# ma-compbio/MATCHA

Measured on AMD Instinct MI355X. Metric: training hyperedges/sec at k∈{2..5}, embed_dim=64; 1/2/4/8 MI355X, higher is better.
Workload: dtype f32; 1 GPU; hg38_1mb bins (N=3067), k in {2,3,4,5} mixed-k zero-padded to L=5, embed_dim=64, front end=table, neg_num=3, dropout on, AdamW lr=1e-3, 400000 known hyperedges; parallelism=dp1, hipgraph=False, table_gradient_exchange=none, embedding_backward=float atomics, exchange_overlapped=False

## Files before the change

### include/matcha_hip.h

```cpp
#ifndef MATCHA_HIP_H
#define MATCHA_HIP_H

#include <stddef.h>
#include <stdint.h>

#ifdef __cplusplus
extern "C" {
#endif

#define MATCHA_ABI_VERSION 7

#define MATCHA_OK 0
#define MATCHA_EINVAL (-22)
#define MATCHA_EHIP (-5)
#define MATCHA_ENOMEM (-12)

#define MATCHA_MAX_L 8
#define MATCHA_MAX_LONG_L 32
#define MATCHA_N_HEAD 8

typedef void* matcha_stream_t;

int matcha_abi_version(void);
const char* matcha_last_error(void);
int matcha_device_count(void);

#define MATCHA_PROF_GEMM_NT 1
#define MATCHA_PROF_GEMM_NN 2
#define MATCHA_PROF_GEMM_TN 3
#define MATCHA_PROF_ATTN_FWD 4
#define MATCHA_PROF_ATTN_BWD 5
#define MATCHA_PROF_EMBED_FWD 6
#define MATCHA_PROF_EMBED_SCATTER 7
#define MATCHA_PROF_LN3_FWD 8
#define MATCHA_PROF_LN3_BWD 9
#define MATCHA_PROF_HEAD_FWD 10
#define MATCHA_PROF_HEAD_BWD 11
#define MATCHA_PROF_ADAMW 12
#define MATCHA_PROF_NEG_SAMPLE 13
#define MATCHA_PROF_ADJ_ENCODE 14
#define MATCHA_PROF_GATHER_ROWS 15
#define MATCHA_PROF_FUSED_FWD 16
#define MATCHA_PROF_FUSED_BWD 17
#define MATCHA_PROF_FRONT_FWD 18
#define MATCHA_PROF_FRONT_BWD 19
#define MATCHA_PROF_ADJ_RECON 20
#define MATCHA_PROF_ADJ_BWD 21
int matcha_profile_select(int32_t kernel_class);
int matcha_profile_read(double* total_ms, int64_t* launches, double* work);

int matcha_launch_log(int32_t on);
int matcha_launch_log_read(char* out, size_t cap);

int matcha_set_option(const char* name, int32_t value);
int32_t matcha_get_option(const char* name);

#define MATCHA_STATUS_BAD_ID 1
#define MATCHA_STATUS_BAD_CHROM 2

typedef struct matcha_shape {
  int32_t d;
  int32_t n_attr;
  int32_t n_nodes;
  int32_t n_chrom;
  int32_t mode;
  int32_t max_bins;
} matcha_shape;

typedef struct matcha_tensors {
  float* table;
  float* adj_w0;
  float* adj_w1;
  float* recon_w;
  float* recon_b;
  float* attr_w;
  float* attr_b;
  float* next_w;
  float* next_b;
  float* ln_q_g; float* ln_q_b;
  float* ln_k_g; float* ln_k_b;
  float* ln_v_g; float* ln_v_b;
  float* w_q;
  float* w_k;
  float* w_v;
  float* fc1_w;
// ... 328 lines not shown
```

### matcha_amd/_lib.py

```python
from __future__ import annotations

import ctypes as C
import os

_HERE = os.path.dirname(os.path.abspath(__file__))
LIB_PATH = os.environ.get("MATCHA_HIP_LIB") or os.path.join(_HERE, "lib", "libmatcha_hip.so")

MAX_L = 8
MAX_LONG_L = 32
N_HEAD = 8

GEMM_NT, GEMM_NN, GEMM_TN = 0, 1, 2
EPI_BIAS, EPI_TANH, EPI_DROPOUT, EPI_ROWMASK, EPI_RESIDUAL, EPI_DTANH, EPI_ACCUM = 1, 2, 4, 8, 16, 32, 64

PROF = dict(gemm_nt=1, gemm_nn=2, gemm_tn=3, attn_fwd=4, attn_bwd=5, embed_fwd=6, embed_scatter=7, ln3_fwd=8, ln3_bwd=9,
            head_fwd=10, head_bwd=11, adamw=12, neg_sample=13, adj_encode=14, gather_rows=15, fused_fwd=16, fused_bwd=17, front_fwd=18, front_bwd=19,
            adj_recon=20, adj_bwd=21)

_fp = C.c_void_p


class Shape(C.Structure):
    _fields_ = [("d", C.c_int32), ("n_attr", C.c_int32), ("n_nodes", C.c_int32), ("n_chrom", C.c_int32),
                ("mode", C.c_int32), ("max_bins", C.c_int32)]
# ... 12 lines not shown
class Frozen(C.Structure):
    _fields_ = [("attr_table", _fp), ("bounds", _fp), ("feats", _fp), ("feat_off", _fp), ("inter", _fp),
                ("bounds_host", _fp), ("feat_row_pad", C.c_int32), ("attr_mode", C.c_int32), ("attr_ld", C.c_int32),
                ("attr_scale", C.c_float), ("attr_bounds", _fp)]


class StepOpts(C.Structure):
    _fields_ = [("training", C.c_int32), ("random_chrom", C.c_int32), ("p_drop_adj", C.c_float),
                ("p_drop_fc1", C.c_float), ("p_drop_pff", C.c_float), ("alpha", C.c_float), ("beta", C.c_float),
                ("seed", _fp), ("forward_only", C.c_int32), ("loss_in_forward", C.c_int32), ("status", _fp),
                ("sparse_table_grad", C.c_int32), ("deterministic", C.c_int32), ("encoder_done_event", _fp),
                ("random_chrom_dev", _fp)]


class RaggedView(C.Structure):
    _fields_ = [("row_off", _fp), ("tok_slot", _fp), ("tok_id", _fp), ("tok_key", _fp), ("tok_pos", _fp), ("count", _fp),
                ("tile_meta", _fp), ("tiles_cap", C.c_int64), ("half_meta", _fp), ("halves_cap", C.c_int64), ("tok_tile", _fp)]


class GemmEpilogue(C.Structure):
    _fields_ = [("flags", C.c_int32), ("bias", _fp), ("residual", _fp), ("aux", _fp), ("row_ids", _fp), ("seed", _fp),
                ("stream_id", C.c_int32), ("p_drop", C.c_float), ("aux_scale", C.c_float)]


_I64, _I32, _SZ, _D, _F = C.c_int64, C.c_int32, C.c_size_t, C.c_double, C.c_float
SIGNATURES = {
    "matcha_abi_version": (C.c_int, []),
    "matcha_last_error": (C.c_char_p, []),
    "matcha_device_count": (C.c_int, []),
    "matcha_profile_select": (C.c_int, [_I32]),
    "matcha_profile_read": (C.c_int, [C.POINTER(C.c_double), C.POINTER(C.c_int64), C.POINTER(C.c_double)]),
    "matcha_launch_log": (C.c_int, [_I32]),
    "matcha_launch_log_read": (C.c_int, [C.c_char_p, _SZ]),
    "matcha_workspace_bytes": (_SZ, [C.POINTER(Shape), _I64, _I32]),
    "matcha_workspace_bytes_forward": (_SZ, [C.POINTER(Shape), _I64, _I32]),
    "matcha_forward": (C.c_int, [C.POINTER(Shape), C.POINTER(Tensors), C.POINTER(Frozen), C.POINTER(StepOpts), _fp, _I64,
                                 _I32, _fp, _fp, _fp, _fp, _fp, _SZ, _fp]),
    "matcha_workspace_bytes_long": (_SZ, [C.POINTER(Shape), _I64, _I32]),
    "matcha_forward_long": (C.c_int, [C.POINTER(Shape), C.POINTER(Tensors), C.POINTER(Frozen), C.POINTER(StepOpts), _fp, _I64,
                                      _I32, _fp, _fp, _fp, _SZ, _fp]),
    "matcha_get_embedding_long": (C.c_int, [C.POINTER(Shape), C.POINTER(Tensors), C.POINTER(Frozen), C.POINTER(StepOpts), _fp, _I64, _I32,
                                            _fp, _fp, _fp, _fp, _fp, _SZ, _fp]),
    "matcha_workspace_bytes_long_train": (_SZ, [C.POINTER(Shape), _I64, _I32]),
    "matcha_forward_long_train": (C.c_int, [C.POINTER(Shape), C.POINTER(Tensors), C.POINTER(Frozen), C.POINTER(StepOpts), _fp, _I64,
                                            _I32, _fp, _fp, _fp, _SZ, _fp]),
    "matcha_backward_long": (C.c_int, [C.POINTER(Shape), C.POINTER(Tensors), C.POINTER(Frozen), C.POINTER(StepOpts), _fp, _I64,
                                       _I32, _fp, _fp, C.POINTER(Tensors), _fp, _fp, _SZ, _fp]),
    "matcha_attn_long_bwd_workspace_bytes": (_SZ, [_I64, _I32]),
    "matcha_attn_long_bwd": (C.c_int, [_fp, _fp, _fp, _fp, _fp, _I64, _I32, _I32, _I32, _fp, _fp, _fp, _fp, _SZ, _fp]),
    "matcha_backward": (C.c_int, [C.POINTER(Shape), C.POINTER(Tensors), C.POINTER(Frozen), C.POINTER(StepOpts), _fp, _I64,
                                  _I32, _fp, _fp, _fp, _fp, C.POINTER(Tensors), _fp, _fp, _SZ, _fp]),
    "matcha_forward_objective": (C.c_int, [_I32, C.POINTER(Shape), C.POINTER(Tensors), C.POINTER(Frozen), C.POINTER(StepOpts), _fp, _I64,
                                           _I32, _fp, _fp, _fp, _fp, _fp, _SZ, _fp]),
    "matcha_backward_objective": (C.c_int, [_I32, C.POINTER(Shape), C.POINTER(Tensors), C.POINTER(Frozen), C.POINTER(StepOpts), _fp, _I64,
                                            _I32, _fp, _fp, _fp, _fp, C.POINTER(Tensors), _fp, _fp, _SZ, _fp]),
    "matcha_node_embeddings": (C.c_int, [C.POINTER(Shape), C.POINTER(Tensors), C.POINTER(Frozen), _fp, _I64, _fp, _fp, _SZ, _fp, _fp]),
    "matcha_get_embedding": (C.c_int, [C.POINTER(Shape), C.POINTER(Tensors), C.POINTER(Frozen), C.POINTER(StepOpts), _fp, _I64, _I32,
                                       _fp, _fp, _fp, _fp, _fp, _SZ, _fp]),
    "matcha_table_grad_rows": (C.c_int, [C.POINTER(Shape), _I64, _I32, _fp, _SZ, C.POINTER(C.c_void_p), C.POINTER(C.c_void_p),
                                         C.POINTER(C.c_void_p), C.POINTER(C.c_int64)]),
    "matcha_scatter_rows_workspace_bytes": (_SZ, [_I64, _I32, _I32]),
    "matcha_scatter_rows": (C.c_int, [_fp, _fp, _I64, _I32, _I32, _fp, _fp, _SZ, _fp]),
    "matcha_ragged_plan_bytes": (_SZ, [_I64, _I32]),
    "matcha_ragged_plan": (C.c_int, [_fp, _I64, _I32, _I32, _fp, _fp, _SZ, C.POINTER(RaggedView), _fp]),
    "matcha_random_chrom_dev_supported": (C.c_int, [C.POINTER(Shape), C.POINTER(Frozen)]),
    "matcha_set_option": (C.c_int, [C.c_char_p, _I32]),
# ... 137 lines not shown
    return old


class option:

    def __init__(self, name: str, value: int = 1):
        self.name, self.value = name, value

    def __enter__(self):
        self.old = set_option(self.name, self.value)
        return self

    def __exit__(self, *a):
        set_option(self.name, self.old)


class launch_log:

    def __enter__(self):
        self.counts = {}
        check(load().matcha_launch_log(1), "matcha_launch_log")
        return self

    def __exit__(self, *a):
        lib = load()
        lib.matcha_launch_log(0)
        buf = C.create_string_buffer(1 << 14)
        check(lib.matcha_launch_log_read(buf, len(buf)), "matcha_launch_log_read")
        for line in buf.value.decode().splitlines():
            name, n = line.rsplit(" ", 1)
            self.counts[name] = int(n)


def raise_on_status(status_host, what: str):
    if status_host[0] & STATUS_BAD_ID:
        raise IndexError(f"{what}: node id outside [0, n_nodes] (the reference's nn.Embedding raises 'index out of range in self')")
    if status_host[0] & STATUS_BAD_CHROM:
        raise KeyError(f"{what}: a node without a chromosome (node2chrom < 0) reached the negative sampler")
```

### matcha_amd/csrc/fused_fwd32.hip

```cpp
#include "kernels.hpp"
#include "prep_heads.hpp"
#include "ragged_roles.hpp"

#ifndef F32_ABL
#define F32_ABL 0
#endif

namespace matcha {

typedef float f32x16 __attribute__((ext_vector_type(16)));

namespace {

constexpr int kLdH = 68;
constexpr int kHT = 32 * kLdH;
constexpr float kEps32 = 1e-5f;
constexpr int kTailVec32 = 2 * 4096;
constexpr int kTailSlab32 = 2 * 4096 + 10 * 64;

struct FL { f32x16 lo, hi; };

__device__ __forceinline__ float xhalf_sum(float v) {
  float a = v, b = v;
  asm volatile("s_nop 1\n\tv_permlane32_swap_b32 %0, %1" : "+v"(a), "+v"(b));
// ... 158 lines not shown
  } while (0)

__device__ __forceinline__ FL fl_zero() {
  FL v;
#pragma unroll
  for (int e = 0; e < 16; ++e) { v.lo[e] = 0.f; v.hi[e] = 0.f; }
  return v;
}

}

__global__ __launch_bounds__(256) void prep_heads_kernel(PrepArgs a) {
  __shared__ __attribute__((aligned(16))) float sm[kPrepLdsFloats];
  prep_heads_role(a, blockIdx.x, blockIdx.y, blockIdx.z, sm);
}

struct Fwd32Args {
  const float* X;
  const int32_t* xrow;
  const int32_t* row_off; const int32_t* tok_slot; const int32_t* count; const int32_t* half_meta; const int32_t* tok_pos;
  int L;
  const u32x4* wfrag;
  HeadParams hp;
  const float* y; const float* w;
  float* Y; float* H1; float* H2;
  float* logits; float* row_loss;
  const uint64_t* seed;
  float p_fc1, p_pff;
  float* ddyn0; float* dXs; float* tslab; float alpha_over_B;
  int objective;
  float* qkv;
  float* tail_dh2;
  const float* rn;
  int rn_rows;
  float* dxs_node;
};

template <int ML>
__global__ __launch_bounds__(64) __attribute__((amdgpu_waves_per_eu(2, 2))) void fused_fwd32_kernel(Fwd32Args g) {
  extern __shared__ __attribute__((aligned(16))) float lds[];
#ifdef FF_TIMING
  long long tph[16] = {0};
  long long tlast = wall_clock64();
#define FF_T(i) do { const long long now__ = wall_clock64(); tph[i] += now__ - tlast; tlast = now__; } while (0)
#else
#define FF_T(i) do { } while (0)
#endif
  float* TK = lds;
  float* TV = lds + kHT;
  float* outs = lds + 2 * kHT;
  float* douts = outs + 32;
  const int lane = threadIdx.x, r = lane & 31, h = lane >> 5;

  const int4 meta = reinterpret_cast<const int4*>(g.half_meta)[blockIdx.x];
  const int t0 = meta.x, n = meta.y, b0 = meta.z, n_h = meta.w;
  if (n_h <= 0) return;
  const int tok_pad = g.count[1];
  const float inv_temp = 0.125f;
  const bool real = r < n;

  const u32x4* wp;
  u32x4 W_[F32_WIN];
  W32_PRIME_AT(g.rn ? 2 : 0);
  {
    const f32x4* bsrc = reinterpret_cast<const f32x4*>(g.wfrag + (kNMat + 1) * kFragU4);
    for (int i4 = lane; i4 < kNBias * 16; i4 += 64) reinterpret_cast<f32x4*>(TV)[i4] = bsrc[i4];
  }
#define F32_BIAS(ROW) fl_vec(TV + (ROW) * 64 + 4 * h)

  int64_t xoff = F32_ROW();
  if (g.xrow) xoff = (int64_t)g.xrow[F32_TOK()] * 64 + 4 * h;
  FL xh = fl_load(g.X + xoff);
  int pos = 0, k = 0;
  if (real) {
    const int tp = g.tok_pos[F32_TOK()];
    pos = tp & 255; k = tp >> 8;
  }
  const int li0 = r - pos;
  float rx;
  {
    float mean;
    fl_stats(xh, mean, rx);
#pragma unroll
    for (int e = 0; e < 16; ++e) { xh.lo[e] = (xh.lo[e] - mean) * rx; xh.hi[e] = (xh.hi[e] - mean) * rx; }
  }
  constexpr int kRec = kImgRecH;
  float* const img_base = g.qkv ? g.qkv + (int64_t)blockIdx.x * MATCHA_N_HEAD * kImgRecH : nullptr;
  const bool img_on = g.qkv != nullptr && real;
#define F32_IMG_STORE(ACC, HD, M)                                                                        \
  do {                                                                                                   \
    if (img_on && !(F32_ABL & 2)) {                                                                      \
      int l__ = lane;                                                                                    \
      asm volatile("" : "+v"(l__));                                                                      \
      f32x4* d__ = reinterpret_cast<f32x4*>(img_base + (HD) * kRec + (M) * 4096 + l__ * 4);             \
      _Pragma("unroll") for (int g__ = 0; g__ < 4; ++g__) {                                              \
        if (F32_ABL & 16) {                                                                              \
          d__[g__ * 64] = (f32x4){ACC.lo[4 * g__], ACC.lo[4 * g__ + 1], ACC.lo[4 * g__ + 2], ACC.lo[4 * g__ + 3]};   \
          d__[(4 + g__) * 64] = (f32x4){ACC.hi[4 * g__], ACC.hi[4 * g__ + 1], ACC.hi[4 * g__ + 2], ACC.hi[4 * g__ + 3]}; \
        } else {                                                                                         \
        __builtin_nontemporal_store((f32x4){ACC.lo[4 * g__], ACC.lo[4 * g__ + 1], ACC.lo[4 * g__ + 2], ACC.lo[4 * g__ + 3]}, d__ + g__ * 64); \
        __builtin_nontemporal_store((f32x4){ACC.hi[4 * g__], ACC.hi[4 * g__ + 1], ACC.hi[4 * g__ + 2], ACC.hi[4 * g__ + 3]}, d__ + (4 + g__) * 64); \
// ... 35 lines not shown
        p[j__] = a__;                                                                                    \
        F32_PIN1(p[j__]);                                                                                \
      }                                                                                                  \
    }                                                                                                    \
    if constexpr ((S) == 2 * (ML + 1)) {                                                                 \
      float mx__ = -3.4e38f;                                                                             \
      _Pragma("unroll") for (int i__ = 0; i__ < ML; ++i__) mx__ = (i__ < k) ? fmaxf(mx__, p[i__]) : mx__; \
      mx__ = hpad ? fmaxf(mx__, p[ML]) : mx__;                                                           \
      float den__ = 0.f;                                                                                 \
      _Pragma("unroll") for (int i__ = 0; i__ < ML; ++i__) { p[i__] = (i__ < k) ? __expf(p[i__] - mx__) : 0.f; den__ += p[i__]; } \
      p[ML] = hpad ? __expf(p[ML] - mx__) : 0.f;                                                         \
      den__ += padf * p[ML];                                                                             \
      const float inv__ = __builtin_amdgcn_rcpf(den__);                                                  \
      _Pragma("unroll") for (int i__ = 0; i__ <= ML; ++i__) { p[i__] *= inv__; F32_PIN1(p[i__]); }       \
    }                                                                                                    \
    if constexpr ((S) == 2 * (ML + 1) + 1) {                                                             \
       \
      if (img_on && h == 0) {                                                                            \
        float wv__[8];                                                                                   \
        _Pragma("unroll") for (int i__ = 0; i__ < 8; ++i__) wv__[i__] = i__ < ML ? p[i__ < ML ? i__ : 0] : 0.f; \
        if (hpad) wv__[7] = p[ML];                                                                       \
        int l__ = lane;                                                                                  \
        asm volatile("" : "+v"(l__));                                                                    \
        f32x4* dst__ = reinterpret_cast<f32x4*>(img_base + hd * kRec + 2048 + (l__ & 31) * 8);          \
        __builtin_nontemporal_store((f32x4){wv__[0], wv__[1], wv__[2], wv__[3]}, dst__);                 \
        __builtin_nontemporal_store((f32x4){wv__[4], wv__[5], wv__[6], wv__[7]}, dst__ + 1);             \
      }                                                                                                  \
    }                                                                                                    \
  } while (0)
#define F32_STAGE8(MAC) do { MAC(0); MAC(1); MAC(2); MAC(3); MAC(4); MAC(5); MAC(6); MAC(7); } while (0)

  FF_T(0);
  fl_store(krow, xh);
  FL dyn;
  if (!g.rn) {
  B3 xs[4];
  FL_SPLIT(xs[0], xh, 0); FL_SPLIT(xs[1], xh, 1); FL_SPLIT(xs[2], xh, 2); FL_SPLIT(xs[3], xh, 3);
  F32_WAVE_SYNC();
  dyn = F32_BIAS(kBiasDyn);
  {
    FL q = F32_BIAS(kBiasR), o;
    W32_CHAIN_XS(q, xs, true);
    F32_IMG_STORE(q, 0, 0);
    FF_T(1);
#define F32_Z_PIECE(S)                                                                                   \
  do {                                                                                                   \
    constexpr int j__ = (S) >> 1, hf__ = (S) & 1;                                                        \
    if constexpr (j__ <= ML) {                                                                           \
      const float* rp__ = TK + ro[j__] + 32 * hf__;                                                      \
      const float w__ = j__ < ML ? p[j__] : padf * p[ML];                                                \
      const f2 w2__ = {w__, w__};                                                                        \
      f32x16& oo__ = hf__ ? o.hi : o.lo;                                                                 \
      _Pragma("unroll") for (int g__ = 0; g__ < 4; ++g__) {                                              \
        const f32x4 a__ = *reinterpret_cast<const f32x4*>(rp__ + 8 * g__);                               \
        const f2 u0__ = __builtin_elementwise_fma(w2__, (f2){a__.x, a__.y}, (f2){oo__[4 * g__], oo__[4 * g__ + 1]});     \
        const f2 u1__ = __builtin_elementwise_fma(w2__, (f2){a__.z, a__.w}, (f2){oo__[4 * g__ + 2], oo__[4 * g__ + 3]}); \
        oo__[4 * g__] = u0__.x; oo__[4 * g__ + 1] = u0__.y; oo__[4 * g__ + 2] = u1__.x; oo__[4 * g__ + 3] = u1__.y;      \
      }                                                                                                  \
      asm volatile("" : "+v"(oo__));                                                                     \
    }                                                                                                    \
  } while (0)
#define F32_MG_PIECE(Q)                                                                                  \
  do {                                                                                                   \
    if constexpr ((F32_ABL & 1) != 0) { } else                                                           \
    if constexpr ((Q) < 2 * (ML + 1) + 2) F32_SC_PIECE(Q); else F32_Z_PIECE((Q) - (2 * (ML + 1) + 2));   \
  } while (0)
#define F32_MG_ONLY(S) do { F32_MG_PIECE(5 * (S)); F32_MG_PIECE(5 * (S) + 1); F32_MG_PIECE(5 * (S) + 2); F32_MG_PIECE(5 * (S) + 3); F32_MG_PIECE(5 * (S) + 4); } while (0)
#define F32_MG_STEP(S) do { WB_MMA(acc, xs[(S) >> 1], S); F32_MG_ONLY(S); WB_REFILL(S, true); } while (0)
    int hd = 0;
    for (; hd + 1 < MATCHA_N_HEAD; ++hd) {
      o = fl_zero();
      {
        FL acc = F32_BIAS(kBiasR + hd + 1);
        F32_STAGE8(F32_MG_STEP);
        q = acc;
        F32_IMG_STORE(q, hd + 1, 0);
      }
      FF_T(2);
      W32_CHAIN(dyn, o, true);
      FF_T(5);
    }
    o = fl_zero();
    F32_STAGE8(F32_MG_ONLY);
    FF_T(2);
    W32_CHAIN(dyn, o, true);
    FF_T(5);
  }
  } else {
    F32_WAVE_SYNC();
    dyn = F32_BIAS(kBiasDyn);
    int roff = g.xrow[F32_TOK()] * 64 + 4 * h;
    const float* rnh = g.rn;
    FL q = fl_load(rnh + roff), o;
    FF_T(1);
    int hd = 0;
    for (; hd + 1 < MATCHA_N_HEAD; ++hd) {
      o = fl_zero();
      rnh += (int64_t)g.rn_rows * 64;
      const FL acc = fl_load(rnh + roff);
      F32_STAGE8(F32_MG_ONLY);
      FF_T(2);
      W32_CHAIN(dyn, o, false);
      W32_PRIME_AT(hd + 1 < MATCHA_N_HEAD - 1 ? 2 * hd + 4 : 15);
      q = acc;
      FF_T(5);
    }
    o = fl_zero();
    F32_STAGE8(F32_MG_ONLY);
    FF_T(2);
    W32_CHAIN(dyn, o, true);
    FF_T(5);
  }
  if (F32_ABL & 8) { if (dyn.lo[0] == 12345.f) g.logits[0] = dyn.hi[3]; return; }
#define F32_XH_RELOAD() do { xh = fl_load(krow); } while (0)
#define F32_TAIL_SYNC() F32_WAVE_SYNC()
#define F32_PARK_Y(V) do { if (g.Y) fl_store_global(g.Y + F32_ROW(), V); } while (0)
#define F32_PARK_H1(V) do { if (g.H1) fl_store_global(g.H1 + F32_ROW(), V); } while (0)
#define F32_UNPARK_Y() fl_unpark(g.Y, F32_ROW())
#define F32_UNPARK_H1() fl_unpark(g.H1, F32_ROW())
#define F32_PARK_HH(V) do { if (g.H2) fl_store_global(g.H2 + F32_ROW(), V); } while (0)
#define F32_UNPARK_HH() fl_unpark(g.H2, F32_ROW())
#define F32_DXS_OUT(V)                                                                                   \
  do {                                                                                                   \
    if (g.dxs_node) {                                                                                    \
      const int key__ = g.xrow[F32_TOK()];                                                               \
      F32_TAIL_SYNC();                                                                                   \
      fl_store(myrow, V);                                                                                \
      F32_TAIL_SYNC();                                                                                   \
      float v__ = T1[lane];                            \
      for (int i__ = 0; i__ < n; ++i__) {                                                                \
        const float vn__ = T1[(i__ + 1 < n ? i__ + 1 : i__) * kLdH + lane];                              \
        const int k__ = __builtin_amdgcn_readlane(key__, i__);                                           \
        unsafeAtomicAdd(g.dxs_node + (int64_t)k__ * 64 + lane, v__);                                     \
        v__ = vn__;                                                                                      \
      }                                                                                                  \
    } else if (r <= n) fl_store_global(g.dXs + F32_ROW(), V);                                            \
  } while (0)
#include "fused_fwd32_tail.hpp"
#undef F32_DXS_OUT
#undef F32_TAIL_SYNC
#undef F32_PARK_Y
#undef F32_PARK_H1
#undef F32_UNPARK_Y
#undef F32_UNPARK_H1
#undef F32_PARK_HH
#undef F32_UNPARK_HH
#ifdef FF_TIMING
  if (blockIdx.x == 2000 && lane == 0)
    printf("fused_fwd32 wave 2000 us: setup %.1f prologue K0 Q0 %.1f | 8 heads: V+scores %.1f K'+PV %.1f Q' %.1f fc1 %.1f | pff fwd %.1f ln+logit %.1f | ln-bwd+colsums %.1f dW1 %.1f dZ1 %.1f dW0 %.1f ddyn %.1f\n",
           tph[0] * 0.01, tph[1] * 0.01, tph[2] * 0.01, tph[3] * 0.01, tph[4] * 0.01, tph[5] * 0.01, tph[7] * 0.01, tph[8] * 0.01, tph[9] * 0.01,
           tph[10] * 0.01, tph[11] * 0.01, tph[12] * 0.01, tph[13] * 0.01);
#endif
}

template <int ML>
__global__ __launch_bounds__(512) void fused_fwd32h_kernel(Fwd32Args g) {
  extern __shared__ __attribute__((aligned(16))) float lds[];
#undef FF_T
#define FF_T(i) do { } while (0)
  float* TK = lds;
  float* TV = lds + kHT;
  float* outs = lds + 2 * kHT;
  float* douts = outs + 32;
  float* Pd = lds + 2 * kHT + 64;
  const int lane = threadIdx.x & 63, r = lane & 31, h = lane >> 5;
  const int hd = __builtin_amdgcn_readfirstlane(threadIdx.x >> 6);

  const int4 meta = reinterpret_cast<const int4*>(g.half_meta)[blockIdx.x];
  const int t0 = meta.x, n = meta.y, b0 = meta.z, n_h = meta.w;
  if (n_h <= 0) return;
  const int tok_pad = g.count[1];
  const float inv_temp = 0.125f;
  const bool real = r < n;

  const u32x4* wp;
  u32x4 W_[F32_WIN];
  W32_PRIME_AT(hd == 0 ? 0 : 2 * hd - 1);
#undef F32_BIAS
#define F32_BIAS(ROW) fl_vec(reinterpret_cast<const float*>(g.wfrag + (kNMat + 1) * kFragU4) + (ROW) * 64 + 4 * h)

  FL xh = fl_load(g.X + F32_ROW());
  int pos = 0, k = 0;
  if (real) {
    const int tp = g.tok_pos[F32_TOK()];
    pos = tp & 255; k = tp >> 8;
  }
  const int li0 = r - pos;
  float rx;
  {
    float mean;
    fl_stats(xh, mean, rx);
#pragma unroll
// ... 121 lines not shown
static int fwd32h_max_halves() { return 2 * device_cu_count(); }

bool fused_small_batch(const Ragged& rg) { return rg.nhalves <= fwd32h_max_halves() && !options().disable_small_batch; }

size_t fused_frag_floats() { return (size_t)(kNMat + 1) * kFragU4 * 4 + (size_t)kNBias * 64; }
size_t fused_tail_slab32_floats(int64_t B, int L) { return (size_t)(ragged_halves_cap(B, L) + 2) * kTailSlab32; }

size_t fused_merged_floats() { return (size_t)2 * MATCHA_N_HEAD * 4096 + MATCHA_N_HEAD * 64 + 64; }
MergedView merged_view(const float* m) {
  return MergedView{m, m + (size_t)MATCHA_N_HEAD * 4096, m + (size_t)2 * MATCHA_N_HEAD * 4096, m + (size_t)2 * MATCHA_N_HEAD * 4096 + MATCHA_N_HEAD * 64};
}
void prep_heads_args(const matcha_tensors& p, float* folded, float* merged, float* frag, PrepArgs& a) {
  const size_t wsz = (size_t)MATCHA_N_HEAD * 64 * 64, csz = (size_t)MATCHA_N_HEAD * 64;
  a.Wq = p.w_q; a.Wk = p.w_k; a.Wv = p.w_v;
  a.gq = p.ln_q_g; a.gk = p.ln_k_g; a.gv = p.ln_v_g; a.bq = p.ln_q_b; a.bv = p.ln_v_b;
  a.fc1_w = p.fc1_w; a.fc1_b = p.fc1_b; a.p0w = p.pff0_w; a.p0b = p.pff0_b; a.p1w = p.pff1_w; a.p1b = p.pff1_b;
  a.fwq = folded; a.fwk = folded + wsz; a.fwv = folded + 2 * wsz; a.fcq = folded + 3 * wsz; a.fcv = a.fcq + 2 * csz;
  const MergedView v = merged_view(merged);
  a.B = const_cast<float*>(v.B); a.M = const_cast<float*>(v.M); a.bvec = const_cast<float*>(v.bvec); a.bdyn = const_cast<float*>(v.bdyn);
  a.frag = reinterpret_cast<u32x4*>(frag);
}
int launch_prep_heads(const matcha_tensors& p, float* folded, float* merged, float* frag, hipStream_t st) {
  PrepArgs a;
  prep_heads_args(p, folded, merged, frag, a);
  hipLaunchKernelGGL(prep_heads_kernel, dim3(kPrepGridX, kPrepGridY, kPrepGridZ), dim3(256), 0, st, a);
  MATCHA_CHECK_LAUNCH("prep_heads_kernel");
  return MATCHA_OK;
}

int launch_fused_fwd32(const matcha_tensors& p, const Ragged& rg, int64_t B, int L, const FusedFwdLaunch& a, hipStream_t st) {
  Fwd32Args g;
  g.xrow = a.x.xrow;
  MATCHA_CHECK_ARG(!a.x.rn || a.x.xrow, "fused forward: the r table belongs to the node route");
  g.rn = a.x.rn; g.rn_rows = (int)a.x.rows;
  g.tail_dh2 = nullptr; g.dxs_node = nullptr;
  g.X = a.x.X; g.row_off = rg.row_off; g.tok_slot = rg.tok_slot; g.count = rg.count; g.half_meta = rg.half_meta; g.tok_pos = rg.tok_pos;
  g.L = L;
  g.wfrag = reinterpret_cast<const u32x4*>(a.frag);
  g.hp = HeadParams{p.pff_ln_g, p.pff_ln_b, p.ln1_g, p.ln1_b, p.ln2_g, p.ln2_b, p.cls_w, p.cls_b};
  const bool target = a.objective == MATCHA_OBJECTIVE_SOFTPLUS_MSE ? a.y != nullptr : (a.y && a.w);
  g.objective = a.objective;
  g.y = a.y; g.w = a.w; g.Y = a.Y; g.H1 = a.H1; g.H2 = a.H2; g.logits = a.logits; g.row_loss = target ? a.row_loss : nullptr;
  g.seed = a.seed; g.p_fc1 = a.p_fc1; g.p_pff = a.p_pff;
  g.ddyn0 = target ? a.ddyn0 : nullptr; g.dXs = a.dXs; g.tslab = a.tslab; g.alpha_over_B = a.alpha / (float)B; g.qkv = a.rimg;
  ProfScope ps(MATCHA_PROF_FUSED_FWD, (double)(B * L + 1) * (MATCHA_N_HEAD * 4.0 + 2.0) * 2.0 * 64.0 * 64.0, st);
  if (a.small) {
    MATCHA_CHECK_ARG(!a.x.xrow, "fused forward: the node route runs the large-batch kernel only");
    const size_t ldsh = ((size_t)10 * kHT + 64) * sizeof(float);
    dispatch_ml(L, [&](auto ml) {
      auto kfn = fused_fwd32h_kernel<decltype(ml)::value>;
      (void)hipFuncSetAttribute(reinterpret_cast<const void*>(kfn), hipFuncAttributeMaxDynamicSharedMemorySize, (int)ldsh);
      hipLaunchKernelGGL(kfn, dim3(rg.nhalves), dim3(512), ldsh, st, g);
    });
    MATCHA_CHECK_LAUNCH("fused_fwd32h_kernel");
    return MATCHA_OK;
  }
  g.tail_dh2 = g.ddyn0 ? a.tail_dh2 : nullptr;
  MATCHA_CHECK_ARG(!a.dxs_node || (a.x.xrow && g.ddyn0), "fused forward: per-node dXs sums belong to the node route with the tail's backward in the kernel");
  g.dxs_node = a.dxs_node;
  const size_t lds = ((size_t)2 * kHT + 64) * sizeof(float);
  dispatch_ml(L, [&](auto ml) { hipLaunchKernelGGL(fused_fwd32_kernel<decltype(ml)::value>, dim3(rg.nhalves), dim3(64), lds, st, g); });
  MATCHA_CHECK_LAUNCH("fused_fwd32_kernel");
  return MATCHA_OK;
}

}
```

### matcha_amd/csrc/layerwise.hpp

```cpp
#pragma once
#include <unordered_map>
#include <utility>

#include "kernels.hpp"

namespace matcha {

int adj_forward(const matcha_shape& s, const matcha_tensors& p, const matcha_frozen& f, const matcha_step_opts& o, const int64_t* x, int64_t T,
                float* node_out, float* recon_out, void* ws, size_t ws_bytes, hipStream_t st, const int32_t* t_dev, const int32_t* slot_map,
                float* fused_x0 = nullptr, float* fused_X = nullptr, bool save = false, bool fused_node = false);
int adj_backward(const matcha_shape& s, const matcha_tensors& p, const matcha_frozen& f, const matcha_step_opts& o, const int64_t* x, int64_t T,
                 float* dnode, const float* drecon, matcha_tensors& g, int32_t* touched, void* ws, size_t ws_bytes, void* gemm_ws,
                 size_t gemm_ws_bytes, hipStream_t st, const int32_t* slot_map, bool fused = false);
size_t adj_workspace_bytes(const matcha_shape& s, int64_t T);

struct TokenChain {
  Ragged rg;
  float *x0, *X, *qin, *kin, *vin, *stats, *Q, *K, *V, *P, *O, *Y, *H1, *H2, *row_loss, *logits, *node;
  float *dH2, *dXs, *dZ1, *ddyn0, *dO, *dQ, *dK, *dV, *dqin, *dkin, *dvin, *dZ0, *dX0;
  float* slab;      size_t slab_bytes;
  float* gemm_ws;   size_t gemm_ws_bytes;
  void* adj_ws;     size_t adj_ws_bytes;
  void* tg_ws;      size_t tg_ws_bytes;
  float *lwB, *lwM, *lwdB, *lwdM;
// ... 2 lines not shown

struct ChainOpts {
  bool merged;
  bool long_attn;
  bool keep;
};

struct ChainCall {
  const matcha_shape& s; const matcha_tensors& p; const matcha_frozen& f; const matcha_step_opts& o;
  int64_t B; int L; hipStream_t st; ChainOpts c; const char* fn;
  int64_t Tn() const { return B * L + 1; }
};

GemmArgs gemm1(const TokenChain& w, const float* A, const float* B, float* C, int64_t M, int64_t N, int64_t K, bool b_kn = false);
int merged_weights(const matcha_shape& s, const matcha_tensors& p, const TokenChain& w, hipStream_t st);
int merged_chain(const matcha_shape& s, const matcha_tensors& p, matcha_tensors& g, const TokenChain& w, hipStream_t st);
void chain_scratch_bytes(const matcha_shape& s, int64_t B, int L, bool long_attn, TokenChain& w);
int check_shape_fields(const matcha_shape* s, const char* fn);
int check_chain_params(const matcha_tensors& p, const matcha_frozen& f, const char* fn);

int chain_front_fwd(const ChainCall& c, const TokenChain& w, float* recon_out, bool zero_recon);
int chain_attn_fwd(const ChainCall& c, const TokenChain& w);
int chain_tail_fwd(const ChainCall& c, const TokenChain& w, const float* y, const float* w_bce, float* logits, float* losses, int objective,
                   bool stop_before_head);
int chain_tail_bwd(const ChainCall& c, const TokenChain& w, const float* X, const int32_t* xrow, const float* y, const float* w_bce, const float* dlogits,
                   int objective, matcha_tensors& g);
int chain_attn_bwd(const ChainCall& c, const TokenChain& w, matcha_tensors& g);
int chain_front_bwd(const ChainCall& c, const TokenChain& w, const float* drecon, matcha_tensors& g, int32_t* touched);

int table_gradient(const matcha_shape& s, const matcha_step_opts& o, const TokenChain& w, int64_t Tn, matcha_tensors& g, hipStream_t st);
int encoder_done(const matcha_step_opts& o, hipStream_t st, const char* fn = "matcha_backward");
void nan_check(const char* name, const float* p, const int32_t* rows_dev, int64_t rows, int64_t width, hipStream_t st);

struct StepRoute {
  bool compact;
  bool half_plan;
  bool fused;
  bool merged_layerwise, enc128;
  bool front, adj_fused;
  bool small;
  bool lif;
  bool split_tail, dx_zeroed;
  bool node;
  bool node_r, node_v;
  bool node_dx;
  bool paired;
  bool long_rows;
};
extern std::unordered_map<const void*, std::pair<StepRoute, uint64_t>> g_fwd_state;
void note_forward(const void* ws, const StepRoute& route);
bool recorded_route(const void* ws, StepRoute& route);
void forget_forward(const void* ws);

}
```

### matcha_amd/csrc/model.hip

```cpp
#include <stdlib.h>
#include <string.h>

#include <unordered_map>

#include "layerwise.hpp"
#include "tail_reduce.hpp"
#include "fb_unfold.hpp"
#include "ragged_roles.hpp"

namespace matcha {

thread_local char g_err[512] = "";
void set_error(const char* fmt, ...) {
  va_list ap;
  va_start(ap, fmt);
  vsnprintf(g_err, sizeof(g_err), fmt, ap);
  va_end(ap);
}

int device_cu_count() {
  static int cache[64] = {};
  int dev = 0;
  if (hipGetDevice(&dev) != hipSuccess) { (void)hipGetLastError(); return 256; }
  if (dev >= 0 && dev < 64 && cache[dev] > 0) return cache[dev];
// ... 142 lines not shown
  w.tslab2 = take(s.d == 64 ? tail_bwd_slab_floats() : 0);
  w.qkv = take(s.d == 64 ? fused_qkv_floats(B, L) : 0);
  w.front_ws = take(front_bwd_supported(s.d, s.n_attr) ? front_bwd_ws_floats() : 0);
  w.tg_ws_bytes = (s.mode == 0 && !compact) ? table_grad_ws_bytes(Tn, s.n_nodes) : 0;
  w.tg_ws = take(w.tg_ws_bytes / sizeof(float));
  {
    const size_t nn = node_front_shape(s, B, L) ? (size_t)(s.n_nodes + 1) : 0;
    w.XN = take_always(nn * 64); w.x0N = take(nn * 64); w.xhN = take(nn * 64); w.GN = take(nn * 64);
    w.node_ids = reinterpret_cast<int64_t*>(take_always(nn * 2));
    w.node_cnt = reinterpret_cast<int32_t*>(take_always(nn ? 64 : 0));
    w.RN = nn ? (compact ? take_always(node_r_floats((int64_t)nn)) : w.Q) : nullptr;
    w.VN = (nn && !compact && w.Q) ? w.Q + node_r_floats((int64_t)nn) : nullptr;
  }
  w.total = off;
  return off;
}

static bool compact_forward(const matcha_shape& s, const matcha_step_opts& o, bool force_layerwise) { return !force_layerwise && o.forward_only && fused_enabled(s); }
static StepRoute decide_route(const matcha_shape& s, const matcha_step_opts& o, int64_t B, int L, const Workspace& w, const matcha_frozen& f,
                              const float* y, const float* w_bce, int objective, bool force_layerwise, bool want_losses) {
  StepRoute r;
  r.compact = compact_forward(s, o, force_layerwise);
  r.fused = !force_layerwise && fused_enabled(s);
  r.merged_layerwise = merged_layerwise(s);
  r.enc128 = !force_layerwise && enc128_enabled(s, o) && (o.forward_only || enc128_rec_floats(w.rg) <= w.enc_rec_floats);
  r.half_plan = fused_enabled(s) || r.enc128;
  r.front = r.fused && front_bwd_supported(s.d, s.n_attr) && (options().disable_fused & 2) == 0;
  r.adj_fused = r.front && s.mode == 1 && adj_fused_eligible(s, f);
  r.small = r.fused && fused_small_batch(w.rg);
  const bool atomics = !o.deterministic && !o.sparse_table_grad;
  r.node = r.front && node_front_shape(s, B, L) && !r.small && atomics && !options().disable_node_front;
  r.node_r = r.node && !options().disable_node_r;
  r.node_v = r.node_r && !o.forward_only && w.VN && node_v_shape(s, B, L) && !options().disable_node_v;
  r.lif = r.fused && o.loss_in_forward && !o.forward_only && has_target(objective, y, w_bce);
  r.split_tail = r.lif && !r.small && (options().fused_dbg & 1) == 0;
  r.dx_zeroed = r.lif && atomics && (r.split_tail || r.small) && want_losses;
  r.node_dx = r.node_v && r.lif && r.split_tail && r.dx_zeroed && node_dx_shape(s, B, L) && !options().disable_node_dx;
  r.paired = r.fused && !options().disable_launch_pairs;
  r.long_rows = false;
  return r;
}
static NodeOperands node_operands(const StepRoute& r, const matcha_shape& s, const Workspace& w) {
  const int64_t rows = (int64_t)s.n_nodes + 1;
  return r.node ? NodeOperands{w.XN, w.rg.tok_key, w.xhN, r.node_r ? w.RN : nullptr, r.node_v ? w.VN : nullptr, rows} : NodeOperands{w.X, nullptr, nullptr, nullptr, nullptr, rows};
}

static int check_shape(const matcha_shape* s, int64_t B, int32_t L) {
  MATCHA_TRY(check_shape_fields(s, nullptr));
  MATCHA_CHECK_ARG(L >= 1 && L <= MATCHA_MAX_L, "L=%d outside 1..%d", L, MATCHA_MAX_L);
  MATCHA_CHECK_ARG(B >= 1 && B * (int64_t)L < (1ll << 31) - 2, "B=%lld must be >= 1 and B*L < 2^31", (long long)B);
  MATCHA_CHECK_ARG(s->d == 64 || B * (int64_t)L + 1 <= 65535ll * 128, "B*L=%lld exceeds the %lld token rows the layer-by-layer kernels (embed_dim != 64) launch",
                   (long long)(B * (int64_t)L), 65535ll * 128);
  return MATCHA_OK;
}

}

using namespace matcha;

extern "C" int matcha_abi_version(void) { return MATCHA_ABI_VERSION; }
extern "C" const char* matcha_last_error(void) { return g_err; }
extern "C" int matcha_device_count(void) {
  int n = 0;
  if (hipGetDeviceCount(&n) != hipSuccess) { (void)hipGetLastError(); return 0; }
  return n;
}

extern "C" int matcha_profile_select(int32_t kernel_class) {
  g_prof_class = kernel_class;
  g_prof_used = 0;
  g_prof_work = 0.0;
  return MATCHA_OK;
}

extern "C" int matcha_launch_log(int32_t on) {
  if (on) g_launch_names = 0;
  g_launch_log = on ? 1 : 0;
  return MATCHA_OK;
}

extern "C" int matcha_launch_log_read(char* out, size_t cap) {
  MATCHA_CHECK_ARG(out && cap > 0, "matcha_launch_log_read: null buffer");
  size_t n = 0;
  out[0] = 0;
  for (int i = 0; i < g_launch_names; ++i) {
    const int k = snprintf(out + n, cap - n, "%s %lld\n", g_launches[i].name, (long long)g_launches[i].n);
    if (k < 0 || (size_t)k >= cap - n) { set_error("matcha_launch_log_read: buffer too small"); return MATCHA_ENOMEM; }
    n += (size_t)k;
  }
  return MATCHA_OK;
}

extern "C" int matcha_profile_read(double* total_ms, int64_t* launches, double* work) {
  double ms = 0.0;
  for (int i = 0; i + 1 < g_prof_used; i += 2) {
    if (hipEventSynchronize(g_prof_ev[i + 1]) != hipSuccess) { set_error("matcha_profile_read: event sync failed"); return MATCHA_EHIP; }
    float t = 0.f;
    if (hipEventElapsedTime(&t, g_prof_ev[i], g_prof_ev[i + 1]) != hipSuccess) { set_error("matcha_profile_read: elapsed failed"); return MATCHA_EHIP; }
    ms += t;
  }
  if (total_ms) *total_ms = ms;
  if (launches) *launches = g_prof_used / 2;
  if (work) *work = g_prof_work;
  g_prof_used = 0;
  g_prof_work = 0.0;
  return MATCHA_OK;
}

extern "C" size_t matcha_workspace_bytes(const matcha_shape* shp, int64_t B, int32_t L) {
  if (check_shape(shp, B, L) != MATCHA_OK) return 0;
  Workspace w;
  return carve(*shp, B, L, nullptr, w);
}

extern "C" size_t matcha_workspace_bytes_forward(const matcha_shape* shp, int64_t B, int32_t L) {
  if (check_shape(shp, B, L) != MATCHA_OK) return 0;
  Workspace w;
  return carve(*shp, B, L, nullptr, w, fused_enabled(*shp));
}

static int forward_impl(const matcha_shape* shp, const matcha_tensors* params, const matcha_frozen* frozen,
                        const matcha_step_opts* opts, const int64_t* x, int64_t B, int32_t L, const float* y,
// ... 289 lines not shown
```

Before: 59.33 million hyperedges/s.

## Read per-node value table in fused forward and restructure attention head loop

Adds a path to the fused f32 forward kernel that loads precomputed per-node value projections (vn) alongside the r table, skipping the per-token value matmul. It also restructures the token and node-r paths to compute value tiles into LDS per head, interleaved with the score pieces. Bias is read from global/L2 (btab) instead of being staged into LDS up front. A route-readout API is added for inspection. The weight-prefetch schedule changes and register pressure may rise. The diff does not show where the caller sets vn in the kernel arguments, so the new path may not be active.

```diff
diff --git a/include/matcha_hip.h b/include/matcha_hip.h
--- a/include/matcha_hip.h
+++ b/include/matcha_hip.h
@@ -51,6 +51,8 @@
 
 int matcha_launch_log(int32_t on);
 int matcha_launch_log_read(char* out, size_t cap);
+
+int matcha_route_read(const void* ws, char* out, size_t cap);
 
 int matcha_set_option(const char* name, int32_t value);
 int32_t matcha_get_option(const char* name);
diff --git a/matcha_amd/_lib.py b/matcha_amd/_lib.py
--- a/matcha_amd/_lib.py
+++ b/matcha_amd/_lib.py
@@ -68,6 +68,7 @@
     "matcha_profile_read": (C.c_int, [C.POINTER(C.c_double), C.POINTER(C.c_int64), C.POINTER(C.c_double)]),
     "matcha_launch_log": (C.c_int, [_I32]),
     "matcha_launch_log_read": (C.c_int, [C.c_char_p, _SZ]),
+    "matcha_route_read": (C.c_int, [_fp, C.c_char_p, _SZ]),
     "matcha_workspace_bytes": (_SZ, [C.POINTER(Shape), _I64, _I32]),
     "matcha_workspace_bytes_forward": (_SZ, [C.POINTER(Shape), _I64, _I32]),
     "matcha_forward": (C.c_int, [C.POINTER(Shape), C.POINTER(Tensors), C.POINTER(Frozen), C.POINTER(StepOpts), _fp, _I64,
@@ -271,6 +272,12 @@
             self.counts[name] = int(n)
 
 
+def route_record(ws) -> dict:
+    buf = C.create_string_buffer(1 << 10)
+    check(load().matcha_route_read(ptr(ws), buf, len(buf)), "matcha_route_read")
+    return {name: int(v) for name, v in (line.rsplit(" ", 1) for line in buf.value.decode().splitlines())}
+
+
 def raise_on_status(status_host, what: str):
     if status_host[0] & STATUS_BAD_ID:
         raise IndexError(f"{what}: node id outside [0, n_nodes] (the reference's nn.Embedding raises 'index out of range in self')")
diff --git a/matcha_amd/csrc/fused_fwd32.hip b/matcha_amd/csrc/fused_fwd32.hip
--- a/matcha_amd/csrc/fused_fwd32.hip
+++ b/matcha_amd/csrc/fused_fwd32.hip
@@ -214,6 +214,7 @@
   float* qkv;
   float* tail_dh2;
   const float* rn;
+  const float* vn;
   int rn_rows;
   float* dxs_node;
 };
@@ -243,12 +244,9 @@
 
   const u32x4* wp;
   u32x4 W_[F32_WIN];
-  W32_PRIME_AT(g.rn ? 2 : 0);
-  {
-    const f32x4* bsrc = reinterpret_cast<const f32x4*>(g.wfrag + (kNMat + 1) * kFragU4);
-    for (int i4 = lane; i4 < kNBias * 16; i4 += 64) reinterpret_cast<f32x4*>(TV)[i4] = bsrc[i4];
-  }
+  const float* const btab = reinterpret_cast<const float*>(g.wfrag + (kNMat + 1) * kFragU4);
 #define F32_BIAS(ROW) fl_vec(TV + (ROW) * 64 + 4 * h)
+#define F32_BIAS_L2(ROW) fl_vec(btab + (ROW) * 64 + 4 * h)
 
   int64_t xoff = F32_ROW();
   if (g.xrow) xoff = (int64_t)g.xrow[F32_TOK()] * 64 + 4 * h;
@@ -350,17 +348,23 @@
 
   FF_T(0);
   fl_store(krow, xh);
-  FL dyn;
-  if (!g.rn) {
-  B3 xs[4];
-  FL_SPLIT(xs[0], xh, 0); FL_SPLIT(xs[1], xh, 1); FL_SPLIT(xs[2], xh, 2); FL_SPLIT(xs[3], xh, 3);
-  F32_WAVE_SYNC();
-  dyn = F32_BIAS(kBiasDyn);
-  {
-    FL q = F32_BIAS(kBiasR), o;
-    W32_CHAIN_XS(q, xs, true);
-    F32_IMG_STORE(q, 0, 0);
-    FF_T(1);
+#define F32_Y_PIECE(S)                                                                                   \
+  do {                                                                                                   \
+    constexpr int j__ = (S) >> 1, hf__ = (S) & 1;                                                        \
+    if constexpr (j__ <= ML) {                                                                           \
+      const float* rp__ = TV + ro[j__] + 32 * hf__;                                                      \
+      const float w__ = j__ < ML ? p[j__] : padf * p[ML];                                                \
+      const f2 w2__ = {w__, w__};                                                                        \
+      f32x16& oo__ = hf__ ? dyn.hi : dyn.lo;                                                             \
+      _Pragma("unroll") for (int g__ = 0; g__ < 4; ++g__) {                                              \
+        const f32x4 a__ = *reinterpret_cast<const f32x4*>(rp__ + 8 * g__);                               \
+        const f2 u0__ = __builtin_elementwise_fma(w2__, (f2){a__.x, a__.y}, (f2){oo__[4 * g__], oo__[4 * g__ + 1]});     \
+        const f2 u1__ = __builtin_elementwise_fma(w2__, (f2){a__.z, a__.w}, (f2){oo__[4 * g__ + 2], oo__[4 * g__ + 3]}); \
+        oo__[4 * g__] = u0__.x; oo__[4 * g__ + 1] = u0__.y; oo__[4 * g__ + 2] = u1__.x; oo__[4 * g__ + 3] = u1__.y;      \
+      }                                                                                                  \
+      asm volatile("" : "+v"(oo__));                                                                     \
+    }                                                                                                    \
+  } while (0)
 #define F32_Z_PIECE(S)                                                                                   \
   do {                                                                                                   \
     constexpr int j__ = (S) >> 1, hf__ = (S) & 1;                                                        \
@@ -378,57 +382,114 @@
       asm volatile("" : "+v"(oo__));                                                                     \
     }                                                                                                    \
   } while (0)
+#define F32_V_PIECE(S) F32_Y_PIECE(S)
+#define F32_NSC (2 * (ML + 1) + 2)
 #define F32_MG_PIECE(Q)                                                                                  \
   do {                                                                                                   \
     if constexpr ((F32_ABL & 1) != 0) { } else                                                           \
-    if constexpr ((Q) < 2 * (ML + 1) + 2) F32_SC_PIECE(Q); else F32_Z_PIECE((Q) - (2 * (ML + 1) + 2));   \
+    if constexpr ((Q) < F32_NSC) F32_SC_PIECE(Q); else F32_V_PIECE((Q) - F32_NSC);                       \
   } while (0)
 #define F32_MG_ONLY(S) do { F32_MG_PIECE(5 * (S)); F32_MG_PIECE(5 * (S) + 1); F32_MG_PIECE(5 * (S) + 2); F32_MG_PIECE(5 * (S) + 3); F32_MG_PIECE(5 * (S) + 4); } while (0)
-#define F32_MG_STEP(S) do { WB_MMA(acc, xs[(S) >> 1], S); F32_MG_ONLY(S); WB_REFILL(S, true); } while (0)
-    int hd = 0;
-    for (; hd + 1 < MATCHA_N_HEAD; ++hd) {
-      o = fl_zero();
+#define F32_MG_STEP(S)                                                                                   \
+  do {                                                                                                   \
+    WB_MMA(acc, xs[(S) >> 1], S);                                                                        \
+    F32_MG_PIECE(5 * (S)); F32_MG_PIECE(5 * (S) + 1); F32_MG_PIECE(5 * (S) + 2);                         \
+    __builtin_amdgcn_sched_barrier(0);                                                                   \
+    F32_MG_PIECE(5 * (S) + 3); F32_MG_PIECE(5 * (S) + 4);                                                \
+    WB_REFILL(S, true);                                                                                  \
+  } while (0)
+#define F32_XS_STEP(S) do { WB_MMA(acc, xs[(S) >> 1], S); WB_REFILL(S, true); } while (0)
+#define F32_SC_ONLY(Q) do { if constexpr ((Q) < F32_NSC) F32_MG_PIECE(Q); } while (0)
+#define F32_R_STEP(S) do { WB_MMA(racc, xs[(S) >> 1], S); F32_SC_ONLY(3 * (S)); F32_SC_ONLY(3 * (S) + 1); F32_SC_ONLY(3 * (S) + 2); WB_REFILL(S, true); } while (0)
+#define F32_Y_STEP(S)                                                                                    \
+  do {                                                                                                   \
+    WB_MMA(acc, xs[(S) >> 1], S);                                                                        \
+    F32_MG_PIECE(F32_NSC + 3 * (S)); F32_MG_PIECE(F32_NSC + 3 * (S) + 1); F32_MG_PIECE(F32_NSC + 3 * (S) + 2);                                          \
+    WB_REFILL(S, true);                                                                                  \
+  } while (0)
+#define F32_STAGE8_TO(MAC, NEXT, MID4, MID6) do { MAC(0); MAC(1); MAC(2); MAC(3); MID4; MAC(4); MAC(5); wp = g.wfrag + (NEXT) * kFragU4; MID6; MAC(6); MAC(7); } while (0)
+#define F32_Y_TILE(V) do { F32_WAVE_SYNC(); fl_store(vrow, V); F32_WAVE_SYNC(); } while (0)
+  FL dyn, q;
+  if (g.vn) {
+    F32_WAVE_SYNC();
+    dyn = F32_BIAS_L2(kBiasDyn);
+    const int roff = g.xrow[F32_TOK()] * 64 + 4 * h;
+    const float *rnh = g.rn, *vnh = g.vn;
+    q = fl_load(rnh + roff);
+    {
+      const FL y0 = fl_load(vnh + roff);
+      fl_store(vrow, y0);
+    }
+    F32_WAVE_SYNC();
+    FF_T(1);
+    for (int hd = 0; hd + 1 < MATCHA_N_HEAD; ++hd) {
+      rnh += (int64_t)g.rn_rows * 64; vnh += (int64_t)g.rn_rows * 64;
+      const FL racc = fl_load(rnh + roff), acc = fl_load(vnh + roff);
+      F32_STAGE8(F32_MG_ONLY);
+      F32_Y_TILE(acc);
+      q = racc;
+      FF_T(2);
+    }
+    W32_PRIME_AT(16);
+  } else {
+    B3 xs[4];
+    FL_SPLIT(xs[0], xh, 0); FL_SPLIT(xs[1], xh, 1); FL_SPLIT(xs[2], xh, 2); FL_SPLIT(xs[3], xh, 3);
+    F32_WAVE_SYNC();
+    if (g.rn) {
+      const int roff = g.xrow[F32_TOK()] * 64 + 4 * h;
+      const float* rnh = g.rn;
+      W32_PRIME_AT(2);
+      q = fl_load(rnh + roff);
       {
-        FL acc = F32_BIAS(kBiasR + hd + 1);
-        F32_STAGE8(F32_MG_STEP);
-        q = acc;
-        F32_IMG_STORE(q, hd + 1, 0);
+        FL acc = fl_zero();
+        F32_STAGE8_TO(F32_XS_STEP, 4, , );
+        fl_store(vrow, acc);
       }
-      FF_T(2);
-      W32_CHAIN(dyn, o, true);
-      FF_T(5);
+      F32_WAVE_SYNC();
+      dyn = F32_BIAS_L2(kBiasDyn);
+      FF_T(1);
+      for (int hd = 0; hd + 1 < MATCHA_N_HEAD; ++hd) {
+        rnh += (int64_t)g.rn_rows * 64;
+        FL acc = fl_zero();
+        F32_STAGE8_TO(F32_MG_STEP, hd < 5 ? 2 * hd + 6 : 10 + hd, q = fl_load(rnh + roff), );
+        F32_Y_TILE(acc);
+        FF_T(2);
+      }
+    } else {
+      W32_PRIME_AT(0);
+      q = F32_BIAS_L2(kBiasR);
+      {
+        FL& acc = q;
+        F32_STAGE8_TO(F32_XS_STEP, 2, , );
+      }
+      F32_IMG_STORE(q, 0, 0);
+      {
+        FL acc = fl_zero();
+        F32_STAGE8_TO(F32_XS_STEP, 1, , );
+        fl_store(vrow, acc);
+      }
+      F32_WAVE_SYNC();
+      dyn = F32_BIAS_L2(kBiasDyn);
+      FL racc = F32_BIAS_L2(kBiasR + 1);
+      FF_T(1);
+      for (int hd = 0; hd + 1 < MATCHA_N_HEAD; ++hd) {
+        F32_STAGE8_TO(F32_R_STEP, hd < 6 ? 2 * hd + 4 : 15, , );
+        F32_IMG_STORE(racc, hd + 1, 0);
+        q = racc;
+        FL acc = fl_zero();
+        F32_STAGE8_TO(F32_Y_STEP, hd < 6 ? 2 * hd + 3 : 16, , racc = F32_BIAS_L2(kBiasR + hd + 2));
+        F32_Y_TILE(acc);
+        FF_T(2);
+      }
     }
-    o = fl_zero();
+  }
+  {
+    constexpr int hd = MATCHA_N_HEAD - 1;
     F32_STAGE8(F32_MG_ONLY);
-    FF_T(2);
-    W32_CHAIN(dyn, o, true);
     FF_T(5);
   }
-  } else {
-    F32_WAVE_SYNC();
-    dyn = F32_BIAS(kBiasDyn);
-    int roff = g.xrow[F32_TOK()] * 64 + 4 * h;
-    const float* rnh = g.rn;
-    FL q = fl_load(rnh + roff), o;
-    FF_T(1);
-    int hd = 0;
-    for (; hd + 1 < MATCHA_N_HEAD; ++hd) {
-      o = fl_zero();
-      rnh += (int64_t)g.rn_rows * 64;
-      const FL acc = fl_load(rnh + roff);
-      F32_STAGE8(F32_MG_ONLY);
-      FF_T(2);
-      W32_CHAIN(dyn, o, false);
-      W32_PRIME_AT(hd + 1 < MATCHA_N_HEAD - 1 ? 2 * hd + 4 : 15);
-      q = acc;
-      FF_T(5);
-    }
-    o = fl_zero();
-    F32_STAGE8(F32_MG_ONLY);
-    FF_T(2);
-    W32_CHAIN(dyn, o, true);
-    FF_T(5);
-  }
+  F32_WAVE_SYNC();
+  if (lane < 32) reinterpret_cast<f32x4*>(TV + kBiasConv0 * 64)[lane] = reinterpret_cast<const f32x4*>(btab + kBiasConv0 * 64)[lane];
   if (F32_ABL & 8) { if (dyn.lo[0] == 12345.f) g.logits[0] = dyn.hi[3]; return; }
 #define F32_XH_RELOAD() do { xh = fl_load(krow); } while (0)
 #define F32_TAIL_SYNC() F32_WAVE_SYNC()
@@ -476,6 +537,8 @@
   extern __shared__ __attribute__((aligned(16))) float lds[];
 #undef FF_T
 #define FF_T(i) do { } while (0)
+#undef F32_V_PIECE
+#define F32_V_PIECE(S) F32_Z_PIECE(S)
   float* TK = lds;
   float* TV = lds + kHT;
   float* outs = lds + 2 * kHT;
@@ -663,7 +726,8 @@
   Fwd32Args g;
   g.xrow = a.x.xrow;
   MATCHA_CHECK_ARG(!a.x.rn || a.x.xrow, "fused forward: the r table belongs to the node route");
-  g.rn = a.x.rn; g.rn_rows = (int)a.x.rows;
+  MATCHA_CHECK_ARG(!a.x.vn || a.x.rn, "fused forward: the value table needs the r table");
+  g.rn = a.x.rn; g.vn = a.x.vn; g.rn_rows = (int)a.x.rows;
   g.tail_dh2 = nullptr; g.dxs_node = nullptr;
   g.X = a.x.X; g.row_off = rg.row_off; g.tok_slot = rg.tok_slot; g.count = rg.count; g.half_meta = rg.half_meta; g.tok_pos = rg.tok_pos;
   g.L = L;
diff --git a/matcha_amd/csrc/layerwise.hpp b/matcha_amd/csrc/layerwise.hpp
--- a/matcha_amd/csrc/layerwise.hpp
+++ b/matcha_amd/csrc/layerwise.hpp
@@ -58,6 +58,7 @@
 int encoder_done(const matcha_step_opts& o, hipStream_t st, const char* fn = "matcha_backward");
 void nan_check(const char* name, const float* p, const int32_t* rows_dev, int64_t rows, int64_t width, hipStream_t st);
 
+constexpr int kValuesToken = 1, kValuesNodeProduct = 2, kValuesTable = 3;
 struct StepRoute {
   bool compact;
   bool half_plan;
@@ -69,6 +70,7 @@
   bool split_tail, dx_zeroed;
   bool node;
   bool node_r, node_v;
+  int fwd_values;
   bool node_dx;
   bool paired;
   bool long_rows;
diff --git a/matcha_amd/csrc/model.hip b/matcha_amd/csrc/model.hip
--- a/matcha_amd/csrc/model.hip
+++ b/matcha_amd/csrc/model.hip
@@ -198,6 +198,7 @@
   r.node = r.front && node_front_shape(s, B, L) && !r.small && atomics && !options().disable_node_front;
   r.node_r = r.node && !options().disable_node_r;
   r.node_v = r.node_r && !o.forward_only && w.VN && node_v_shape(s, B, L) && !options().disable_node_v;
+  r.fwd_values = (r.fused && !r.small) ? (r.node_v ? kValuesTable : r.node_r ? kValuesNodeProduct : kValuesToken) : 0;
   r.lif = r.fused && o.loss_in_forward && !o.forward_only && has_target(objective, y, w_bce);
   r.split_tail = r.lif && !r.small && (options().fused_dbg & 1) == 0;
   r.dx_zeroed = r.lif && atomics && (r.split_tail || r.small) && want_losses;
@@ -254,6 +255,21 @@
     if (k < 0 || (size_t)k >= cap - n) { set_error("matcha_launch_log_read: buffer too small"); return MATCHA_ENOMEM; }
     n += (size_t)k;
   }
+  return MATCHA_OK;
+}
+
+extern "C" int matcha_route_read(const void* ws, char* out, size_t cap) {
+  MATCHA_CHECK_ARG(ws && out && cap > 0, "matcha_route_read: null pointer");
+  StepRoute r;
+  MATCHA_CHECK_ARG(recorded_route(ws, r), "matcha_route_read: no forward on record for this workspace");
+  const auto& [compact, half_plan, fused, merged_layerwise, enc128, front, adj_fused, small, lif, split_tail, dx_zeroed, node, node_r, node_v, fwd_values, node_dx,
+               paired, long_rows] = r;
+  const int k = snprintf(out, cap,
+                         "compact %d\nhalf_plan %d\nfused %d\nmerged_layerwise %d\nenc128 %d\nfront %d\nadj_fused %d\nsmall %d\nlif %d\nsplit_tail %d\ndx_zeroed %d\n"
+                         "node %d\nnode_r %d\nnode_v %d\nfwd_values %d\nnode_dx %d\npaired %d\nlong_rows %d\n",
+                         compact, half_plan, fused, merged_layerwise, enc128, front, adj_fused, small, lif, split_tail, dx_zeroed, node, node_r, node_v, fwd_values,
+                         node_dx, paired, long_rows);
+  if (k < 0 || (size_t)k >= cap) { set_error("matcha_route_read: buffer too small"); return MATCHA_ENOMEM; }
   return MATCHA_OK;
 }
 
```

Result: faster. 62.00 million hyperedges/s, median of 6 (+4.5%).
